# jedward225/MARL-HideAndSeek

Measured on AMD Instinct MI355X. Metric: world-steps/sec (agent-steps/sec derived) at 16K worlds, 1/2/4/8 GPU, higher is better.
Workload: dtype f32; 1 GPU; 16000 worlds/GPU x 2646 steps, 2 hiders + 2 seekers, sim_flags=0, rand_seed=0, random move actions in [-5,4] each step (scripts/benchmark.py args); worlds_per_gpu=16000, total_worlds=16000, agents_per_world=4

## Files before the change

### marl-hideandseek_amd/csrc/hs_k_physics.h

```cpp
#pragma once
#include "hs_state.h"
#include "hs_rays.h"
#include "hs_collide.h"
#include "hs_solver.h"
#include "hs_k_reset.h"

namespace hs {

constexpr int kPhysThreads = 64;
constexpr int kWorldLanes = kPhysThreads / kTile;
constexpr int kLdsWalls = 32;
static_assert(kMaxSCand <= 32 && kMaxDDCand <= 16, "accepted-manifold masks are one word per world");
constexpr int kAllDD = kNumDSlots * (kNumDSlots - 1) / 2;
constexpr int kAllSC = kNumDSlots * (kMaxWalls + kMaxPlanes - 1);
constexpr int kSpInfoWords = kNumDSlots + 1;

struct alignas(16) OctRes {
    static constexpr int kClip = kClipLanes;
    static constexpr int kClipWords = clip_words(kClip);
    static constexpr int kSatPairs = kClip < hs::kSatPairs ? kClip : hs::kSatPairs;
    static constexpr int kMaxItems = kTile * (kMaxDDCand + kMaxSCand);
    static constexpr int kSlots = kClip < 31 ? kClip : 31;
    static constexpr int kVelOffsetWords = 2 * 8 * 3 * 32;
    float pos[3][kNumDSlots][kTile];
    float rot[4][kNumDSlots][kTile];
    float ppos[3][kNumDSlots][kTile];
    float prot[4][kNumDSlots][kTile];
    int meta[kNumDSlots][kTile];
    union {
        struct {
            float lo[3][kNumDSlots][kTile], hi[3][kNumDSlots][kTile];
            float wall[4][kLdsWalls][kTile];
        } det;
        struct {
            float clip[kClipWords];
            unsigned short items[kMaxItems + 32];
            int pend[4][kClip];
        } sat;
        struct {
            float pad[kVelOffsetWords];
            float lin[3][kNumDSlots][kTile];
            float ang[3][kNumDSlots][kTile];
        } vel;
    } u;
    unsigned short ddPair[kMaxDDCand][kTile];
    unsigned short scPair[kMaxSCand][kTile];
    unsigned short scInfo[kNumDSlots][kTile];
    unsigned int scAcc[kTile];
    unsigned int ddAcc[kTile];
    unsigned int ddOrd[2][kTile];
    float plane0[4][kTile];
    unsigned char bodies[kNumDSlots * kTile];
    union {
        unsigned char wallBodies[kNumDSlots * kTile];
        unsigned char actGL[kMaxAgents][kTile];
    };
    unsigned int wallSeen[kTile];
    unsigned char numWalls[kTile], numPlanes[kTile], ndd[kTile], nsc[kTile], seen[kTile], hasGrab[kTile];
    unsigned char spill[kTile];
    int wid[kTile];
};
constexpr int kSeenDeferred = 2;
static_assert(sizeof(OctRes) <= 20 * 1024, "8 waves of 8 worlds share the CU's 160 KiB of LDS");
static_assert(offsetof(OctRes, u.sat.items) >= offsetof(OctRes, u.det.wall), "items must not overlap the AABBs");
static_assert(sizeof(ManDD) / 4 * OctRes::kSlots <= OctRes::kVelOffsetWords, "manifold slots lie below the velocities");
static_assert(2 * 3 * kNumDSlots * 8 <= OctRes::kVelOffsetWords, "the hull AABBs lie below the velocities");

constexpr int kLocGlobal = 31;
HSD int pair_a(int p) { return p & 31; }
HSD int pair_b(int p) { return (p >> 5) & 63; }
HSD int pair_loc(int p) { return (p >> 11) & 31; }
HSD int pair_pack(int a, int b) { return a | (b << 5) | (kLocGlobal << 11); }
static_assert(kNumDSlots <= 32 && kMaxWalls + kMaxPlanes <= 64, "pair encoding");
static_assert(sizeof(ManDD) % 16 == 0 && sizeof(ManS) % 16 == 0, "manifold records move 16 bytes at a time");
constexpr int kManWords = sizeof(ManDD) / 4;
template <typename M> HSD void man_lds_load(const float *clip, int slot, M &m) {
    m = *reinterpret_cast<const M *>(clip + slot * kManWords);
}
template <typename M> HSD void man_lds_set_lam(float *clip, int slot, int j, float v) {
    static_assert(offsetof(M, lam) == sizeof(M) - 16, "lam is the record's tail");
    clip[slot * kManWords + (sizeof(M) / 4 - 4 + j)] = v;
}

template <int C> HSD V3 rld3(const float (&a)[C][kNumDSlots][kTile], int slot, int g) { return {a[0][slot][g], a[1][slot][g], a[2][slot][g]}; }
HSD Q rld4(const float (&a)[4][kNumDSlots][kTile], int slot, int g) { return {a[0][slot][g], a[1][slot][g], a[2][slot][g], a[3][slot][g]}; }
HSD void rst3(float (&a)[3][kNumDSlots][kTile], int slot, int g, V3 v) { a[0][slot][g] = v.x; a[1][slot][g] = v.y; a[2][slot][g] = v.z; }
HSD void rst4(float (&a)[4][kNumDSlots][kTile], int slot, int g, Q q) { a[0][slot][g] = q.w; a[1][slot][g] = q.x; a[2][slot][g] = q.y; a[3][slot][g] = q.z; }

HSD void rbody_load(const OctRes &R, int g, int slot, BodyS &b) {
    b.pos = rld3(R.pos, slot, g); b.rot = rld4(R.rot, slot, g);
    b.ppos = rld3(R.ppos, slot, g); b.prot = rld4(R.prot, slot, g);
    b.lin = rld3(R.u.vel.lin, slot, g); b.ang = rld3(R.u.vel.ang, slot, g);
    const int m = R.meta[slot][g];
    const bool dyn = m != 0 && meta_resp(m) == RESP_DYNAMIC;
    b.invM = dyn ? obj_inv_mass(meta_obj(m)) : 0.f;
    b.invI = dyn ? obj_inv_inertia(meta_obj(m)) : V3{0.f, 0.f, 0.f};
    body_refresh_inertia(b);
}
HSD void rbody_store_pose(OctRes &R, int g, int slot, const BodyS &b) { rst3(R.pos, slot, g, b.pos); rst4(R.rot, slot, g, b.rot); }
HSD void rbody_store_vel(OctRes &R, int g, int slot, const BodyS &b) { rst3(R.u.vel.lin, slot, g, b.lin); rst3(R.u.vel.ang, slot, g, b.ang); }
HSD void derive_velocity(BodyS &b) {
    const float h = kSubstepH;
    b.lin = (b.pos - b.ppos) * (1.f / h);
    Q dq = qmul(b.rot, qinv(b.prot));
    V3 wv = V3{dq.x, dq.y, dq.z} * (2.f / h);
    b.ang = dq.w >= 0.f ? wv : -wv;
}

HSD void wave_sync() { asm volatile("s_waitcnt lgkmcnt(0)" ::: "memory"); }
HSD void mem_sync() { asm volatile("s_waitcnt vmcnt(0) lgkmcnt(0)" ::: "memory"); }

template <int D> HSD int dpp_row_shr(int x) { return __builtin_amdgcn_update_dpp(0, x, 0x110 + D, 0xF, 0xF, true); }
HSD int scan8_incl(int x, int l) {
    int y;
    y = dpp_row_shr<1>(x); if (l >= 1) x += y;
    y = dpp_row_shr<2>(x); if (l >= 2) x += y;
    y = dpp_row_shr<4>(x); if (l >= 4) x += y;
    return x;
}
HSD int sum8_all(int x) {
    x += __builtin_amdgcn_update_dpp(0, x, 0xB1, 0xF, 0xF, false);
    x += __builtin_amdgcn_update_dpp(0, x, 0x4E, 0xF, 0xF, false);
    x += __builtin_amdgcn_update_dpp(0, x, 0x141, 0xF, 0xF, false);
    return x;
}
HSD int scan64_incl(int x) {
    x += dpp_row_shr<1>(x); x += dpp_row_shr<2>(x); x += dpp_row_shr<4>(x); x += dpp_row_shr<8>(x);
    x += __builtin_amdgcn_update_dpp(0, x, 0x142, 0xA, 0xF, false);
    x += __builtin_amdgcn_update_dpp(0, x, 0x143, 0xC, 0xF, false);
    return x;
}

struct ResGeom {
    const OctRes &R; const SimState &S; int g; int w;
    HSD int g_meta(int i) const { return R.meta[i][g]; }
    HSD V3 g_pos(int i) const { return rld3(R.pos, i, g); }
    HSD Q g_rot(int i) const { return rld4(R.rot, i, g); }
    HSD int g_num_walls() const { return R.numWalls[g]; }
    HSD float g_wall(int k, int c) const { return S.walls(c * kMaxWalls + k, w); }
    HSD int g_num_planes() const { return R.numPlanes[g]; }
    HSD float g_plane(int p, int c) const { return S.planes(c * kMaxPlanes + p, w); }
};

constexpr float kGroundOff = 0.f;
struct BodyReg {
    int np, vidx;
    float lam[4];
};

template <typename E, int ROWS>
HSD void copy_in(E *dst, const Col<E, ROWS> &col, int p0) {
    static_assert(sizeof(E) == 4, "16-byte pieces");
    const float4 *src = reinterpret_cast<const float4 *>(col.octet(p0 >> 3));
    float4 *d = reinterpret_cast<float4 *>(dst);
    for (int i = hs_lane(); i < ROWS * 2; i += 64) d[i] = src[(i / 2) * 2 + i % 2];
}
template <typename E, int ROWS>
HSD void copy_out(const Col<E, ROWS> &col, int p0, const E *src) {
    static_assert(sizeof(E) == 4, "16-byte pieces");
    float4 *dst = reinterpret_cast<float4 *>(col.octet(p0 >> 3));
    const float4 *s = reinterpret_cast<const float4 *>(src);
    for (int i = hs_lane(); i < ROWS * 2; i += 64) dst[(i / 2) * 2 + i % 2] = s[i];
}
HSD void copy_out_vel(const Col<float, 3 * kNumDSlots> &col, int p0, const float *src, const OctRes &R) {
    float *dst = col.octet(p0 >> 3);
    for (int i = hs_lane(); i < 3 * kNumDSlots * kTile; i += 64) {
        const int row = i / kTile, g = i % kTile, slot = row % kNumDSlots;
        const int m = R.meta[slot][g];
        if (m != 0 && meta_resp(m) == RESP_DYNAMIC) dst[row * kTile + g] = src[i];
    }
}

HSD void integrate_body(OctRes &R, BodyReg &b, int slot, int g, int meta, const float *aforce) {
    const int obj = meta_obj(meta);
    const bool dyn = meta_resp(meta) == RESP_DYNAMIC;
    V3 force = {0.f, 0.f, 0.f}; float torque = 0.f;
    if (dyn && slot >= kAgentSlot0) {
        const float *f = aforce + (slot - kAgentSlot0) * kTile + g;
        force = {f[0 * kMaxAgents * kTile], f[1 * kMaxAgents * kTile], f[2 * kMaxAgents * kTile]};
        torque = f[3 * kMaxAgents * kTile];
    }
    V3 pos = rld3(R.pos, slot, g); Q rot = rld4(R.rot, slot, g);
    rst3(R.ppos, slot, g, pos); rst4(R.prot, slot, g, rot);
    if (dyn) {
        V3 lin = rld3(R.u.vel.lin, slot, g), ang = rld3(R.u.vel.ang, slot, g);
        const float h = kSubstepH;
        const float invM = obj_inv_mass(obj);
        const V3 invI = obj_inv_inertia(obj);
        lin = madd(lin, madd(V3{0.f, 0.f, kGravityZ}, force, invM), h);
        pos = madd(pos, lin, h);
        Q qi = qinv(rot);
        V3 wloc = qrot(qi, ang), tl = qrot(qi, V3{0.f, 0.f, torque});
        const V3 I = obj_inertia(obj);
        V3 Iw = mulc(I, wloc);
        wloc = madd(wloc, mulc(invI, tl - cross(wloc, Iw)), h);
        ang = qrot(rot, wloc);
        rot = quat_add_rotation(rot, ang * h);
        rst3(R.pos, slot, g, pos); rst4(R.rot, slot, g, rot);
        rst3(R.u.vel.lin, slot, g, lin); rst3(R.u.vel.ang, slot, g, ang);
    }
    V3 lo, hi;
    const HullRef hb = hull_ref_body(obj, pos, rot);
    hull_aabb(hb, &lo, &hi);
    rst3(R.u.det.lo, slot, g, lo); rst3(R.u.det.hi, slot, g, hi);
    b.np = 0; b.vidx = 0;
#pragma unroll
    for (int j = 0; j < 4; ++j) b.lam[j] = 0.f;
    if (dyn && R.numPlanes[g] >= 1) {
        const V3 pn = {R.plane0[0][g], R.plane0[1][g], R.plane0[2][g]};
        b.np = ground_manifold(hb, pn, R.plane0[3][g], &b.vidx);
    }
}

struct ItemCounts { int nbox, nwedge; bool anySpill; };
template <int JB>
HSD ItemCounts phase_detect(const SimState &S, OctRes &R, int NS) {
    constexpr int G = kWorldLanes;
    const int L = hs_lane(), g = L / G, l = L % G;
    {
        constexpr int PR = kTile / 4;
        static_assert(kLdsWalls * PR <= 64, "one piece per lane per component");
        const float *src = S.walls.octet(S.wbeg >> 3);
        float4 v[4];
        const bool on = L < kLdsWalls * PR;
        const int row = L / PR, part = L % PR;
#pragma unroll
        for (int c = 0; c < 4; ++c) if (on) v[c] = *(const float4 *)(src + (c * kMaxWalls + row) * kTile + 4 * part);
#pragma unroll
        for (int c = 0; c < 4; ++c) if (on) *(float4 *)(&R.u.det.wall[c][row][4 * part]) = v[c];
    }
    if (l == 0) { R.scAcc[g] = 0u; R.ddAcc[g] = 0u; }
    wave_sync();
    const int nwl = R.numWalls[g], npl = R.numPlanes[g];
    int tot_items = 0;
    unsigned dd_mask[JB] = {}; unsigned long long s_mask[JB] = {};
    int bdd[JB] = {}, bsc[JB] = {}, add[JB] = {}, asc[JB] = {};
    bool have[JB], dynamic[JB]; V3 lo[JB], hi[JB];
#pragma unroll
    for (int jb = 0; jb < JB; ++jb) {
        const int slot = l + jb * G;
        const int meta = slot < NS ? R.meta[slot][g] : 0;
        have[jb] = meta != 0;
        dynamic[jb] = have[jb] && meta_resp(meta) == RESP_DYNAMIC;
        lo[jb] = {0.f, 0.f, 0.f}; hi[jb] = {0.f, 0.f, 0.f};
        if (have[jb]) { lo[jb] = rld3(R.u.det.lo, slot, g); hi[jb] = rld3(R.u.det.hi, slot, g); }
    }
#pragma unroll 4
    for (int j = 1; j < NS; ++j) {
        const int mj = R.meta[j][g];
        const bool dynj = meta_resp(mj) == RESP_DYNAMIC;
        const V3 loj = rld3(R.u.det.lo, j, g), hij = rld3(R.u.det.hi, j, g);
#pragma unroll
        for (int jb = 0; jb < JB; ++jb) {
            const bool hit = (mj != 0) & have[jb] & (l + jb * G < j) & (dynamic[jb] | dynj) &
                (lo[jb].x <= hij.x) & (loj.x <= hi[jb].x) & (lo[jb].y <= hij.y) & (loj.y <= hi[jb].y) &
                (lo[jb].z <= hij.z) & (loj.z <= hi[jb].z);
            dd_mask[jb] |= hit ? 1u << j : 0u;
        }
    }
    bool zin[JB];
#pragma unroll
    for (int jb = 0; jb < JB; ++jb) zin[jb] = dynamic[jb] & (lo[jb].z <= 2.5f) & (0.f <= hi[jb].z);
    auto wall_test = [&](int k, float cx, float cy, float hx, float hy) {
        const float wx0 = cx - hx, wx1 = cx + hx, wy0 = cy - hy, wy1 = cy + hy;
#pragma unroll
        for (int jb = 0; jb < JB; ++jb) {
            const bool hit = zin[jb] & (lo[jb].x <= wx1) & (wx0 <= hi[jb].x) & (lo[jb].y <= wy1) & (wy0 <= hi[jb].y);
            s_mask[jb] |= hit ? 1ull << k : 0ull;
        }
    };
    const int nwLds = nwl < kLdsWalls ? nwl : kLdsWalls;
#pragma unroll 4
    for (int k = 0; k < nwLds; ++k) wall_test(k, R.u.det.wall[0][k][g], R.u.det.wall[1][k][g], R.u.det.wall[2][k][g], R.u.det.wall[3][k][g]);
    for (int k = kLdsWalls; k < nwl; ++k) {
        const int w = S.wbeg + g;
        wall_test(k, S.walls(0 * kMaxWalls + k, w), S.walls(1 * kMaxWalls + k, w), S.walls(2 * kMaxWalls + k, w), S.walls(3 * kMaxWalls + k, w));
    }
    int tot_dd = 0, tot_sc = 0;
#pragma unroll
    for (int jb = 0; jb < JB; ++jb) {
        if (dynamic[jb]) for (int p = 1; p < npl; ++p) s_mask[jb] |= 1ull << (kMaxWalls + p);
        const int cdd = __popc(dd_mask[jb]), csc = __popcll(s_mask[jb]);
        const int in_dd = scan8_incl(cdd, l), in_sc = scan8_incl(csc, l);
        bdd[jb] = tot_dd + in_dd - cdd; bsc[jb] = tot_sc + in_sc - csc;
        tot_dd += sum8_all(cdd); tot_sc += sum8_all(csc);
        add[jb] = cdd ? max(0, min(cdd, kMaxDDCand - bdd[jb])) : 0;
        asc[jb] = csc ? max(0, min(csc, kMaxSCand - bsc[jb])) : 0;
        tot_items += add[jb] + asc[jb];
        if (add[jb] != cdd) atomicAdd(&S.status[0], cdd - add[jb]);
        if (asc[jb] != csc) atomicAdd(&S.status[1], csc - asc[jb]);
    }
    const bool spillDD = tot_dd > kMaxDDCand, spillSC = tot_sc > kMaxSCand;
    const bool anySpill = __ballot(spillDD || spillSC) != 0ull;
    unsigned short *const spPair = S.spPair + (size_t)(S.wbeg + g) * (kAllDD + kAllSC);
    int *const spInfo = S.spInfo + (size_t)(S.wbeg + g) * kSpInfoWords;
    int n_wedge = 0;
#pragma unroll
    for (int jb = 0; jb < JB; ++jb) {
        const int slot = l + jb * G;
        const bool ramp = slot >= kRampSlot0 && slot < kRampSlot0 + kMaxRamps;
        if (ramp) n_wedge += add[jb] + asc[jb];
        else { unsigned mm = dd_mask[jb]; for (int i = 0; mm && i < add[jb]; ++i) { const int j = __ffs(mm) - 1; mm &= mm - 1; n_wedge += (j >= kRampSlot0 && j < kRampSlot0 + kMaxRamps) ? 1 : 0; } }
    }
    const int n_box = tot_items - n_wedge;
    const int inc_box = scan64_incl(n_box), inc_wedge = scan64_incl(n_wedge);
    ItemCounts ic;
    ic.anySpill = anySpill;
    ic.nbox = __builtin_amdgcn_readlane(inc_box, 63); ic.nwedge = __builtin_amdgcn_readlane(inc_wedge, 63);
    const int wedge0 = (ic.nbox + 31) / 32 * 32;
    int ibox = inc_box - n_box, iwedge = wedge0 + inc_wedge - n_wedge;
    wave_sync();
#pragma unroll
    for (int jb = 0; jb < JB; ++jb) {
        const int slot = l + jb * G;
        const bool ramp = slot >= kRampSlot0 && slot < kRampSlot0 + kMaxRamps;
        unsigned mm = dd_mask[jb]; int i = 0;
        while (mm && i < add[jb]) {
            const int j = __ffs(mm) - 1; mm &= mm - 1;
            R.ddPair[bdd[jb] + i][g] = (unsigned short)pair_pack(slot, j);
            const unsigned short item = (unsigned short)((g << 6) | (bdd[jb] + i));
            if (ramp || (j >= kRampSlot0 && j < kRampSlot0 + kMaxRamps)) R.u.sat.items[iwedge++] = item; else R.u.sat.items[ibox++] = item;
            ++i;
        }
        while (mm) {
            const int j = __ffs(mm) - 1; mm &= mm - 1;
            spPair[bdd[jb] + i] = (unsigned short)pair_pack(slot, j);
            ++i;
        }
        unsigned long long sm = (s_mask[jb] >> kMaxWalls) | (s_mask[jb] << (64 - kMaxWalls) >> (64 - kMaxWalls) << kMaxPlanes); i = 0;
        while (sm && i < asc[jb]) {
            const int bit = __ffsll((long long)sm) - 1; sm &= sm - 1;
            const int k = bit < kMaxPlanes ? kMaxWalls + bit : bit - kMaxPlanes;
            R.scPair[bsc[jb] + i][g] = (unsigned short)pair_pack(slot, k);
            const unsigned short item = (unsigned short)((g << 6) | 32 | (bsc[jb] + i));
            if (ramp) R.u.sat.items[iwedge++] = item; else R.u.sat.items[ibox++] = item;
            ++i;
        }
        const int nspill = sm ? __popcll(sm) : 0;
        while (sm) {
            const int bit = __ffsll((long long)sm) - 1; sm &= sm - 1;
            const int k = bit < kMaxPlanes ? kMaxWalls + bit : bit - kMaxPlanes;
            spPair[kAllDD + bsc[jb] + i] = (unsigned short)pair_pack(slot, k);
            ++i;
        }
        if (spillSC && slot < kNumDSlots) spInfo[1 + slot] = nspill ? ((bsc[jb] + asc[jb]) | (nspill << 16)) : 0;
        if (slot < NS) R.scInfo[slot][g] = (unsigned short)(asc[jb] > 0 ? (bsc[jb] | (asc[jb] << 8)) : 0);
    }
    if (l == 0) {
        R.spill[g] = (unsigned char)((spillDD ? 1 : 0) | (spillSC ? 2 : 0));
        if (spillDD || spillSC) spInfo[0] = tot_dd | (tot_sc << 16);
        R.ndd[g] = (unsigned char)min(tot_dd, kMaxDDCand); R.nsc[g] = (unsigned char)min(tot_sc, kMaxSCand);
        if (R.wid[g] >= 0 && tot_dd + tot_sc > 0) S.loadAcc[R.wid[g]] += tot_dd + tot_sc;
    }
    wave_sync();
    return ic;
}

template <bool POS, int UNROLL, typename SetLam>
HSD void static_manifold(BodyS &me, const ManS &m, SetLam set_lam) {
    BodyS none;
    body_refresh_inertia(me);
    const V3 n = ld3(m.n);
    const int np = m.np;
    const float mu = POS ? m.muS : m.muD;
#pragma unroll UNROLL
    for (int j = 0; j < 4; ++j)
        if (j < np) {
            const float lamj = m.lam[j];
            if (POS) set_lam(j, lamj + solve_point_position<false>(me, none, n, ld3(m.rA[j]), V3{0.f, 0.f, 0.f}, m.offB[j], mu));
            else solve_point_velocity<false>(me, none, n, ld3(m.rA[j]), V3{0.f, 0.f, 0.f}, lamj, mu);
        }
}

#define HS_COLD __device__ __forceinline__
struct SpillCtx {
    const float *walls, *planes;
    ManDD *wsDD; ManS *wsSC; unsigned short *spPair; int *spInfo;
    int wbeg;
};
HSD SpillCtx spill_ctx(const SimState &S) { return {S.walls.p, S.planes.p, (ManDD *)S.wsDD, (ManS *)S.wsSC, S.spPair, S.spInfo, S.wbeg}; }

HS_COLD void spill_sat(SpillCtx c, OctRes *Rp) {
    OctRes &R = *Rp;
    const int lane = hs_lane() & 63;
    const bool hi = (lane & 1) != 0;
    const Col<float, 4 * kMaxWalls> walls = {const_cast<float *>(c.walls)};
    const Col<float, 4 * kMaxPlanes> planes = {const_cast<float *>(c.planes)};
#pragma unroll 1
    for (int g = 0; g < kTile; ++g) {
        const int fl = __builtin_amdgcn_readfirstlane((int)R.spill[g]);
        if (fl == 0) continue;
        const int w = c.wbeg + g;
        const int tot = __builtin_amdgcn_readfirstlane(c.spInfo[(size_t)w * kSpInfoWords]);
#pragma unroll 1
        for (int kind = 0; kind < 2; ++kind) {
            if ((fl & (1 << kind)) == 0) continue;
            const bool isdd = kind == 0;
            const int n = isdd ? tot & 0xffff : tot >> 16;
#pragma unroll 1
            for (int base = isdd ? kMaxDDCand : kMaxSCand; base < n; base += OctRes::kSatPairs) {
                const int kk = base + (lane >> 1);
                if (kk < n && (lane >> 1) < OctRes::kSatPairs) {
                    const int pair = c.spPair[(size_t)w * (kAllDD + kAllSC) + (isdd ? 0 : kAllDD) + kk];
                    const int a = pair_a(pair), bsel = pair_b(pair);
                    const int oa = meta_obj(R.meta[a][g]);
                    const V3 pa = rld3(R.pos, a, g);
                    const Q qa = rld4(R.rot, a, g);
                    ManDD *const md = c.wsDD + (size_t)w * kAllDD + kk;
                    ManS *const ms = c.wsSC + (size_t)w * kAllSC + kk;
                    RawManifold raw;
                    raw.np = 0;
                    bool plane = false;
                    if (!isdd && bsel >= kMaxWalls) {
                        const int p = bsel - kMaxWalls;
                        const V3 pn = {planes(0 * kMaxPlanes + p, w), planes(1 * kMaxPlanes + p, w), planes(2 * kMaxPlanes + p, w)};
                        plane = true;
                        if (!hi && !collide_hull_plane(hull_ref_body(oa, pa, qa), pn, planes(3 * kMaxPlanes + p, w), raw)) raw.np = 0;
                    } else {
                        const HullSrc ha = hull_src_body(oa, pa, qa);
                        const HullSrc hb = isdd ? hull_src_body(meta_obj(R.meta[bsel][g]), rld3(R.pos, bsel, g), rld4(R.rot, bsel, g))
                                                : hull_src_wall(walls(0 * kMaxWalls + bsel, w), walls(1 * kMaxWalls + bsel, w),
                                                                walls(2 * kMaxWalls + bsel, w), walls(3 * kMaxWalls + bsel, w));
                        const AxisResult res = sat_axes(ha, hb, hi);
                        const ClipBuf cb = {R.u.sat.clip, lane >> 1, OctRes::kClip};
                        if (!hi && res.code != 0 && !sat_contact(ha, hb, res, cb, raw)) raw.np = 0;
                    }
                    if (!hi) {
                        const int ob = isdd ? meta_obj(R.meta[bsel][g]) : plane ? OBJ_PLANE : OBJ_WALL;
                        const float muS = 0.5f * (obj_mu_s(oa) + obj_mu_s(ob)), muD = 0.5f * (obj_mu_d(oa) + obj_mu_d(ob));
                        const Q qai = qinv(qa);
                        if (isdd) {
                            md->a = a; md->b = bsel; md->np = raw.np; md->muS = muS; md->muD = muD;
                            st3(md->n, raw.n);
                            const V3 pb = rld3(R.pos, bsel, g);
                            const Q qbi = qinv(rld4(R.rot, bsel, g));
#pragma unroll
                            for (int j = 0; j < 4; ++j)
                                if (j < raw.np) {
                                    st3(md->rA[j], qrot(qai, raw.pA[j] - pa)); st3(md->rB[j], qrot(qbi, raw.pB[j] - pb));
                                    md->lam[j] = 0.f;
                                }
                        } else {
                            ms->np = raw.np; ms->muS = muS; ms->muD = muD;
                            st3(ms->n, raw.n);
#pragma unroll
                            for (int j = 0; j < 4; ++j)
                                if (j < raw.np) {
                                    st3(ms->rA[j], plane ? hull_local_vertex(oa, raw.vidx[j]) : qrot(qai, raw.pA[j] - pa));
                                    ms->offB[j] = dot(raw.pB[j], raw.n); ms->lam[j] = 0.f;
                                }
                        }
                    }
                }
                wave_sync();
            }
        }
    }
    mem_sync();
}

template <bool POS>
HS_COLD void spill_dd(SpillCtx c, OctRes *Rp) {
    OctRes &R = *Rp;
#pragma unroll 1
    for (int g = 0; g < kTile; ++g) {
        if ((__builtin_amdgcn_readfirstlane((int)R.spill[g]) & 1) == 0) continue;
        const int w = c.wbeg + g;
        const int nall = __builtin_amdgcn_readfirstlane(c.spInfo[(size_t)w * kSpInfoWords]) & 0xffff;
        if (hs_lane() == 0) {
#pragma unroll 1
            for (int k = kMaxDDCand; k < nall; ++k) {
                ManDD *const m = c.wsDD + (size_t)w * kAllDD + k;
                const int np = m->np;
                if (np <= 0) continue;
                const int ba = m->a, bb = m->b;
                BodyS Ab, Bb;
                rbody_load(R, g, ba, Ab); rbody_load(R, g, bb, Bb);
                const V3 n = ld3(m->n);
                const float mu = POS ? m->muS : m->muD;
#pragma unroll 1
                for (int j = 0; j < np; ++j) {
                    const float lamj = m->lam[j];
                    if (POS) m->lam[j] = lamj + solve_point_position<true>(Ab, Bb, n, ld3(m->rA[j]), ld3(m->rB[j]), 0.f, mu);
                    else solve_point_velocity<true>(Ab, Bb, n, ld3(m->rA[j]), ld3(m->rB[j]), lamj, mu);
                }
                if (POS) { rbody_store_pose(R, g, ba, Ab); rbody_store_pose(R, g, bb, Bb); }
                else { rbody_store_vel(R, g, ba, Ab); rbody_store_vel(R, g, bb, Bb); }
                wave_sync();
            }
        }
    }
}

template <bool POS>
HS_COLD void spill_static(SpillCtx c, OctRes *Rp, int NS) {
    OctRes &R = *Rp;
#pragma unroll 1
    for (int g = 0; g < kTile; ++g) {
        if ((__builtin_amdgcn_readfirstlane((int)R.spill[g]) & 2) == 0) continue;
        const int w = c.wbeg + g;
        const int slot = hs_lane();
        if (slot >= NS) continue;
        const int info = c.spInfo[(size_t)w * kSpInfoWords + 1 + slot];
        const int first = info & 0xffff, cnt = info >> 16;
        if (cnt == 0) continue;
        BodyS me;
        rbody_load(R, g, slot, me);
#pragma unroll 1
        for (int k = first; k < first + cnt; ++k) {
            ManS &m = c.wsSC[(size_t)w * kAllSC + k];
            if (m.np <= 0) continue;
            static_manifold<POS, 1>(me, m, [&](int j, float v) { m.lam[j] = v; });
        }
        if (POS) rbody_store_pose(R, g, slot, me); else rbody_store_vel(R, g, slot, me);
    }
}

HSD HullSrc sat_hull_a(const OctRes &R, int g, int a) { return hull_src_body(meta_obj(R.meta[a][g]), rld3(R.pos, a, g), rld4(R.rot, a, g)); }
HSD HullSrc sat_hull_b(const SimState &S, const OctRes &R, int g, int w, bool isdd, int bsel) {
    if (isdd) return hull_src_body(meta_obj(R.meta[bsel][g]), rld3(R.pos, bsel, g), rld4(R.rot, bsel, g));
    return hull_src_wall(S.walls(0 * kMaxWalls + bsel, w), S.walls(1 * kMaxWalls + bsel, w),
                         S.walls(2 * kMaxWalls + bsel, w), S.walls(3 * kMaxWalls + bsel, w));
}
HSD bool sat_flush(const SimState &S, OctRes &R, int npend, bool last) {
    const int lane = hs_lane() & 63;
    const bool toLds = last && lane < OctRes::kSlots;
    bool wroteGlobal = false;
    int mw[kManWords]; int mkind = 0, mkk = 0, mg = 0, mpair = 0;
    if (lane < npend) {
        const int item = R.u.sat.pend[0][lane] & 0xffff;
        AxisResult res;
        res.code = R.u.sat.pend[0][lane] >> 16;
        res.ax = {__int_as_float(R.u.sat.pend[1][lane]), __int_as_float(R.u.sat.pend[2][lane]), __int_as_float(R.u.sat.pend[3][lane])};
        const int g = item >> 6, idx = item & 63;
        const int w = S.wbeg + g;
        const bool isdd = idx < 32;
        const int kk = idx & 31;
        const int pair = isdd ? R.ddPair[kk][g] : R.scPair[kk][g];
        const int a = pair_a(pair), bsel = pair_b(pair);
        const ClipBuf cb = {R.u.sat.clip, lane, OctRes::kClip};
        RawManifold raw;
        const bool plane = res.code == 3;
        bool have;
        if (plane) {
            const int p = bsel - kMaxWalls;
            const V3 pn = {S.planes(0 * kMaxPlanes + p, w), S.planes(1 * kMaxPlanes + p, w), S.planes(2 * kMaxPlanes + p, w)};
            have = collide_hull_plane(hull_ref_body(meta_obj(R.meta[a][g]), rld3(R.pos, a, g), rld4(R.rot, a, g)), pn, S.planes(3 * kMaxPlanes + p, w), raw);
        } else {
            have = sat_contact(sat_hull_a(R, g, a), sat_hull_b(S, R, g, w, isdd, bsel), res, cb, raw);
        }
        if (have) {
            const int oa = meta_obj(R.meta[a][g]);
            const int ob = isdd ? meta_obj(R.meta[bsel][g]) : plane ? OBJ_PLANE : OBJ_WALL;
            const V3 pa = rld3(R.pos, a, g);
            const Q qai = qinv(rld4(R.rot, a, g));
            const float muS = 0.5f * (obj_mu_s(oa) + obj_mu_s(ob)), muD = 0.5f * (obj_mu_d(oa) + obj_mu_d(ob));
            if (isdd) {
                ManDD m;
                m.a = a; m.b = bsel; m.np = raw.np; m.muS = muS; m.muD = muD;
                st3(m.n, raw.n);
                const V3 pb = rld3(R.pos, bsel, g);
                const Q qbi = qinv(rld4(R.rot, bsel, g));
#pragma unroll
                for (int j = 0; j < 4; ++j) {
                    const bool on = j < raw.np;
                    st3(m.rA[j], on ? qrot(qai, raw.pA[j] - pa) : V3{0.f, 0.f, 0.f});
                    st3(m.rB[j], on ? qrot(qbi, raw.pB[j] - pb) : V3{0.f, 0.f, 0.f});
                    m.lam[j] = 0.f;
                }
                if (toLds) { __builtin_memcpy(mw, &m, sizeof(m)); mkind = 1; mkk = kk; mg = g; mpair = pair; }
                else { ((ManDD *)S.wsDD + (size_t)w * kAllDD)[kk] = m; wroteGlobal = true; }
                atomicOr(&R.ddAcc[g], 1u << kk);
            } else {
                ManS m;
                m.np = raw.np; m.muS = muS; m.muD = muD; m.pad[0] = 0.f; m.pad[1] = 0.f;
                st3(m.n, raw.n);
#pragma unroll
                for (int j = 0; j < 4; ++j) {
                    const bool on = j < raw.np;
// ... 452 lines not shown
                } else if (owner == OWNER_NONE) {
                    R.meta[hit][g] = meta_pack(obj, RESP_STATIC, type == AGENT_HIDER ? OWNER_HIDER : OWNER_SEEKER);
                }
            }
        }
        if (fl & 1) {
            if (S.grabOther(i, w) >= 0) {
                S.grabOther(i, w) = -1;
            } else {
                float t; V3 o = mpos + V3{0.f, 0.f, 0.5f};
                V3 dir = qrot(mrot, {0.f, 1.f, 0.f});
                int hit = trace_ray(geom, o, dir, 2.5f, &t);
                if (hit >= 0 && hit < kNumDSlots) {
                    const int m = R.meta[hit][g];
                    if (meta_owner(m) == OWNER_NONE && meta_resp(m) == RESP_DYNAMIC) {
                        V3 hit_pos = o + dir * t;
                        Q erot = geom.g_rot(hit);
                        V3 r2 = qrot(qinv(erot), hit_pos - geom.g_pos(hit));
                        Q at2 = qnormalize(qmul(qinv(erot), mrot));
                        S.grabOther(i, w) = hit;
                        const float gd[kGrabWords] = {r2.x, r2.y, r2.z, at2.w, at2.x, at2.y, at2.z, t - 1.25f,
                                                      0.f, 1.25f, 0.5f,
                                                      1.f, 0.f, 0.f, 0.f};
#pragma unroll
                        for (int c = 0; c < kGrabWords; ++c) S.grabData(c * kMaxAgents + i, w) = gd[c];
                    }
                }
            }
        }
    }
}

HSD void phase_pre(const SimState &S, OctRes &R) {
    const int A_ = S.A, L = hs_lane();
    const bool instant = (S.flags & FLAG_ZERO_AGENT_VELOCITY) == FLAG_ZERO_AGENT_VELOCITY;
    bool need_action = false;
    if (L < kMaxAgents * kTile) {
        const int agent = L / kTile, g = L % kTile;
        const int w = R.wid[g], p = S.wbeg + g;
        int fl = 0;
        if (agent < A_ && w >= 0) {
            const int teams = S.teams[w], step = S.curEpisodeStep[w];
            const bool active = team_agent_active(teams, agent) != 0;
            const int type = team_agent_type(teams, agent);
            if (active && !(type == AGENT_SEEKER && step < kNumPrepSteps - 1)) {
                int32_t *act_row = S.xAction + (w * A_ + agent) * 5;
                const int ax = act_row[0], ay = act_row[1], ar = act_row[2], ag = act_row[3], al = act_row[4];
                float fx, fy, tz;
                if (instant) { fx = 400.f * (float)(ax - 2); fy = 400.f * (float)(ay - 2); tz = 120.f * (float)(ar - 2); }
                else { fx = 12.f * (float)(ax - 5); fy = 12.f * (float)(ay - 5); tz = 3.f * (float)(ar - 5); }
                V3 f = qrot(rld4(R.rot, kAgentSlot0 + agent, g), {fx, fy, 0.f});
                S.aforce(0 * kMaxAgents + agent, p) = f.x; S.aforce(1 * kMaxAgents + agent, p) = f.y;
                S.aforce(2 * kMaxAgents + agent, p) = f.z; S.aforce(3 * kMaxAgents + agent, p) = tz;
                fl = (ag == 1 ? 1 : 0) | (al == 1 ? 2 : 0);
                act_row[0] = 2; act_row[1] = 2; act_row[2] = 2; act_row[3] = 0; act_row[4] = 0;
            }
        }
        R.actGL[agent][g] = (unsigned char)fl;
        need_action = fl != 0;
    }
    const bool any = __ballot(need_action) != 0ull;
    wave_sync();
    if (any && L < kTile && R.wid[L] >= 0) {
        bool want = false;
        for (int a = 0; a < A_; ++a) want |= R.actGL[a][L] != 0;
        if (want) action_system(S, R, L, A_, S.teams[R.wid[L]]);
    }
    if (L < kTile) {
        bool grab = false;
        if (R.wid[L] >= 0) for (int a = 0; a < kMaxAgents; ++a) grab |= S.grabOther(a, S.wbeg + L) >= 0;
        R.hasGrab[L] = grab ? 1 : 0;
    }
    wave_sync();
}

HSD void phase_post(const SimState &S, OctRes &R) {
    constexpr int G = kWorldLanes;
    const int L = hs_lane(), g = L / G, l = L % G;
    const int w = R.wid[g], p = S.wbeg + g;
    const int A_ = S.A;
    const bool wok = w >= 0;
    const bool instant = (S.flags & FLAG_ZERO_AGENT_VELOCITY) == FLAG_ZERO_AGENT_VELOCITY;
    int teams = 0, step = 0, counts = 0, resetReq = 0;
    float hider_reward = 0.f;
    if (wok) {
        teams = S.teams[w]; step = S.curEpisodeStep[w]; counts = S.counts[w];
        hider_reward = S.hiderTeamReward[w]; resetReq = S.xReset[w];
        if (l == 0) R.seen[g] = 0;
        if (instant && l < kMaxAgents && R.meta[kAgentSlot0 + l][g] != 0) {
            const int slot = kAgentSlot0 + l;
            R.u.vel.lin[0][slot][g] = 0.f; R.u.vel.lin[1][slot][g] = 0.f;
            R.u.vel.lin[2][slot][g] = fminf(R.u.vel.lin[2][slot][g], 0.f);
            rst3(R.u.vel.ang, slot, g, V3{0.f, 0.f, 0.f});
        }
    }
    const bool undecided = wok && step >= kNumPrepSteps - 1 && hider_reward != -1.f;
    const bool defer = undecided && (S.flags & FLAG_EXT_SKIP_OBSERVATIONS) != FLAG_EXT_SKIP_OBSERVATIONS && resetReq == 0 &&
                       !((S.flags & FLAG_IGNORE_EPISODE_LENGTH) != FLAG_IGNORE_EPISODE_LENGTH && step == kEpisodeLen - 1);
    if (defer && l == 0) R.seen[g] = kSeenDeferred;
    wave_sync();
    for (int pr = l; undecided && !defer && pr < 9; pr += G) {
        const int si = pr / 3, hi_ = pr % 3;
        if (si < cnt_seekers(counts) && hi_ < cnt_hiders(counts)) {
            const ResGeom geom = {R, S, g, p};
            const int ss = kAgentSlot0 + team_seeker(teams, si), hs_ = kAgentSlot0 + team_hider(teams, hi_);
            const V3 spos = geom.g_pos(ss);
            const V3 fwd = qrot(geom.g_rot(ss), {0.f, 1.f, 0.f});
            V3 to = geom.g_pos(hs_) - spos;
            float c = dot(normalize(to), fwd);
            if (!(c < kCosFovHalf)) {
                float t;
                if (trace_ray(geom, spos, to, 1.f, &t) == hs_) R.seen[g] = 1;
            }
        }
    }
    wave_sync();
    if (!wok) return;
    if (R.seen[g] == 1) hider_reward = -1.f;
    if (l < A_ && team_agent_active(teams, l)) {
        const int agent = l, slot = kAgentSlot0 + agent, row = w * A_ + agent;
        if (step == 0) S.xDone[row] = 0;
        if (step < kNumPrepSteps - 1) {
            S.xReward[row] = 0.f;
        } else {
            if (step == kEpisodeLen - 1) S.xDone[row] = 1;
            float r = hider_reward;
            if (team_agent_type(teams, agent) == AGENT_SEEKER) r *= -1.f;
            if (fabsf(R.pos[0][slot][g]) >= 18.f || fabsf(R.pos[1][slot][g]) >= 18.f) r -= 10.f;
            S.xReward[row] = r;
        }
    }
    if (l == 0) {
        float *res = S.xEpisodeResult + w * 2;
        int s0 = S.runningScores(0, p), s1 = S.runningScores(1, p);
        if (step == 0) { res[0] = 0.f; res[1] = 0.f; s0 = 0; s1 = 0; }
        if (step >= kNumPrepSteps) {
            const bool hidden = hider_reward == 1.f;
            const bool sf = cnt_seekers_first(counts) != 0;
            const int win = hidden ? (sf ? 1 : 0) : (sf ? 0 : 1);
            if (win == 0) s0 += 1; else s1 += 1;
        }
        if (step == kEpisodeLen - 1) {
            if (s0 > s1) { res[0] = 1.f; res[1] = 0.f; }
            else if (s0 < s1) { res[0] = 0.f; res[1] = 1.f; }
            else { res[0] = 0.5f; res[1] = 0.5f; }
        }
        S.runningScores(0, p) = s0; S.runningScores(1, p) = s1;
        S.hiderTeamReward[w] = hider_reward;
    }
}

template <int ROUNDS, int LASTR, bool POS>
HSD void static_passes(const SimState &S, OctRes &R, BodyReg (&br)[ROUNDS], int nbodies, int nLast, int nMerged) {
    const int L = hs_lane();
#pragma unroll
    for (int r = 0; r < LASTR; ++r) {
        const bool valid = r * 64 + L < nbodies; const int t_ = valid ? R.bodies[r * 64 + L] : 0;
        const int slot = t_ >> 3, g = t_ & 7; const int meta = valid ? R.meta[slot][g] : 0;
        if (valid) { if (POS) ground_pos(R, br[r], slot, g, meta); else ground_vel(R, br[r], slot, g, meta); }
    }
    wave_sync();
    {
        const bool valid = LASTR * 64 + L < nbodies; const int t_ = valid ? R.bodies[LASTR * 64 + L] : 0;
        const int slot = t_ >> 3, g = t_ & 7; const int meta = valid ? R.meta[slot][g] : 0;
        last_round<POS>(S, R, br[LASTR], valid, slot, g, meta, nLast, nMerged);
    }
    wave_sync();
}

#ifdef HS_PHASE_TIMING
#define HS_TICK_PARAMS , long long &tk, long long (&acc)[10]
#define HS_TICK_ARGS , tk, acc
#define HS_TICK(i) { const long long now_ = wall_clock64(); acc[i] += now_ - tk; tk = now_; }
#else
#define HS_TICK_PARAMS
#define HS_TICK_ARGS
#define HS_TICK(i)
#endif
#define HS_BODY(r) const bool valid = (r) * 64 + L < nbodies; const int t_ = valid ? R.bodies[(r) * 64 + L] : 0; \
                   const int slot = t_ >> 3, g = t_ & 7; const int meta = valid ? R.meta[slot][g] : 0;
template <int ROUNDS>
HSD void substep_rest(const SimState &S, OctRes &R, BodyReg (&br)[ROUNDS], int nbodies, int NS, ItemCounts ic, bool integrateNext,
                      const float *aforce HS_TICK_PARAMS) {
    const int L = hs_lane();
    const bool manGlobal = phase_sat(S, R, ic);
    HS_TICK(3)
    phase_dd<true>(S, R, ic.anySpill);
    HS_TICK(4)
    constexpr int kShortLastR = ROUNDS - 2;
    const bool shortLast = ROUNDS == 3 && nbodies <= 64 * (ROUNDS - 1);
    const int lastRound = shortLast ? kShortLastR : ROUNDS - 1;
    const WallLists wl = list_wall_bodies<ROUNDS>(R, nbodies, lastRound);
    const int nLast = max(nbodies - 64 * lastRound, 0);
    const int nMerged = min(wl.nEarly, 64 - nLast);
    if (shortLast) static_passes<ROUNDS, kShortLastR, true>(S, R, br, nbodies, nLast, nMerged);
    else static_passes<ROUNDS, ROUNDS - 1, true>(S, R, br, nbodies, nLast, nMerged);
    if (wl.nwb > nMerged) { wall_round<true>(S, R, nMerged, wl.nwb); wave_sync(); }
    if (__builtin_expect(ic.anySpill, 0)) { spill_static<true>(spill_ctx(S), &R, NS); wave_sync(); }
#pragma unroll
    for (int r = 0; r < ROUNDS; ++r) { HS_BODY(r) if (valid) derive_body_velocity(R, slot, g, meta); }
    if (manGlobal) mem_sync(); else wave_sync();
    HS_TICK(5)
    phase_dd<false>(S, R, ic.anySpill);
    HS_TICK(6)
    if (shortLast) static_passes<ROUNDS, kShortLastR, false>(S, R, br, nbodies, nLast, nMerged);
    else static_passes<ROUNDS, ROUNDS - 1, false>(S, R, br, nbodies, nLast, nMerged);
    if (wl.nwb > nMerged) { wall_round<false>(S, R, nMerged, wl.nwb); wave_sync(); }
    if (__builtin_expect(ic.anySpill, 0)) { spill_static<false>(spill_ctx(S), &R, NS); wave_sync(); }
    if (integrateNext) {
#pragma unroll
        for (int r = 0; r < ROUNDS; ++r) { HS_BODY(r) if (valid) integrate_body(R, br[r], slot, g, meta, aforce); }
        wave_sync();
    }
    HS_TICK(7)
}

template <int ROUNDS>
HSD void physics_step(SimState &S, OctRes &R, GenScratch *gen) {
    const int L = hs_lane();
    const int noct = gridDim.x;
    const int sidx = step_ring(S), prevIdx = sidx == 0 ? 2 : sidx - 1, nextIdx = sidx == 2 ? 0 : sidx + 1;
    const int serve = step_serve(S);
    if (serve != kGroupEarly && blockIdx.x == 0 && L == 0) {
        S.tickSum[nextIdx] = 0ull;
        atomicExch(group_count(S, prevIdx, kGroupEarly), 0); atomicExch(group_count(S, prevIdx, kGroupLate), 0);
    }
    int o = blockIdx.x;
    if (serve != kGroupAll) {
        if (o >= *group_count(S, sidx, serve)) return;
        o = oct_list(S, sidx, serve, noct)[o];
    }
    S.wbeg = o * kTile;
    const int p0 = S.wbeg;
    const int NS = kAgentSlot0 + S.A;
    const long long tStart = wall_clock64();
    int prevTicks, lateAbove;
    {
        prevTicks = S.octTicks[o];
        const float mean = (float)S.tickSum[prevIdx] / (float)noct, mine = (float)prevTicks;
        const bool known = mean > 0.f;
        lateAbove = __builtin_amdgcn_readfirstlane(known ? (int)fminf(2.f * __int_as_float(sched_words(S)[kSchedFactor]) * mean, 2.0e9f) : 0x7fffffff);
        const bool late = serve == kGroupLate;
        if (late && L == 0) atomicAdd(&S.status[2], 1);
        if (known && mine > 1.10f * mean) __builtin_amdgcn_s_setprio(3);
        else if (known && mine > 0.98f * mean) __builtin_amdgcn_s_setprio(2);
        else if ((known && mine > 0.88f * mean) || (known && late)) __builtin_amdgcn_s_setprio(1);
        else if (known) __builtin_amdgcn_s_setprio(0);
        else __builtin_amdgcn_s_setprio(2);
    }
#ifdef HS_PHASE_TIMING
    long long tk = wall_clock64(); long long acc[10] = {0, 0, 0, 0, 0, 0, 0, 0, 0, 0};
#endif
    copy_in(&R.pos[0][0][0], S.bpos, p0); copy_in(&R.rot[0][0][0], S.brot, p0);
    copy_in(&R.u.vel.lin[0][0][0], S.blin, p0); copy_in(&R.u.vel.ang[0][0][0], S.bang, p0);
    copy_in(&R.meta[0][0], S.bmeta, p0);
    if (L < kTile) {
        const int w = S.worldOfSlot[S.wbeg + L];
        R.wid[L] = w;
        R.numWalls[L] = w >= 0 ? (unsigned char)S.numWalls[w] : 0;
        R.numPlanes[L] = w >= 0 ? (unsigned char)S.numPlanes[w] : 0;
        R.seen[L] = 0; R.ndd[L] = 0; R.nsc[L] = 0;
        R.wallSeen[L] = w >= 0 ? (unsigned)S.wallHist[w] : 0u;
    }
    if (L < 4 * kTile) (&R.plane0[0][0])[L] = S.planes((L / kTile) * kMaxPlanes, S.wbeg + (L % kTile));
    wave_sync();
    HS_TICK(9)
    phase_pre(S, R);
    HS_TICK(0)
    int nbodies;
    {
        int base = 0;
#pragma unroll
        for (int pass = 0; pass < 2; ++pass) {
#pragma unroll
            for (int c = 0; c < ROUNDS; ++c) {
                const int t = c * 64 + L;
                const int ord = t / kTile, g = t % kTile;
                const int slot = ord < S.A ? kAgentSlot0 + ord : ord - S.A;
                const bool hist = ord < NS && ((R.wallSeen[g] >> slot) & 1u) != 0u;
                const bool on = ord < NS && R.meta[slot][g] != 0 && hist == (pass == 0);
                const unsigned long long m = __ballot(on);
                if (on) R.bodies[base + __popcll(m & ((1ull << L) - 1ull))] = (unsigned char)(slot << 3 | g);
                base += __popcll(m);
            }
        }
        nbodies = base;
    }
    wave_sync();
    if (L < kTile) R.wallSeen[L] = 0u;
    wave_sync();
    BodyReg br[ROUNDS];
    const float *const aforce = S.aforce.octet(p0 >> 3);
#pragma unroll
    for (int r = 0; r < ROUNDS; ++r) {
        BodyReg &b = br[r];
        b.np = 0; b.vidx = 0;
#pragma unroll
        for (int j = 0; j < 4; ++j) b.lam[j] = 0.f;
        HS_BODY(r)
        if (valid) integrate_body(R, b, slot, g, meta, aforce);
    }
    wave_sync();
    HS_TICK(1)
#pragma unroll 1
    for (int sub = 0; sub < kNumSubsteps; ++sub) {
        const ItemCounts ic = phase_detect<ROUNDS>(S, R, NS);
        HS_TICK(2)
        substep_rest<ROUNDS>(S, R, br, nbodies, NS, ic, sub + 1 < kNumSubsteps, aforce HS_TICK_ARGS);
    }
#undef HS_BODY
    phase_post(S, R);
    wave_sync();
    copy_out(S.bpos, p0, &R.pos[0][0][0]); copy_out(S.brot, p0, &R.rot[0][0][0]);
    copy_out_vel(S.blin, p0, &R.u.vel.lin[0][0][0], R); copy_out_vel(S.bang, p0, &R.u.vel.ang[0][0][0], R);
    copy_out(S.bmeta, p0, &R.meta[0][0]);
    mem_sync();
    HS_TICK(8)
    {
        const int myWorld = L < kTile ? R.wid[L] : -1;
        const int mySeen = L < kTile ? (int)R.wallSeen[L] : 0;
        const bool myDeferred = L < kTile && R.seen[L] == kSeenDeferred;
        wave_sync();
        if (myWorld >= 0) {
            S.wallHist[myWorld] = mySeen;
            reset_world(S, myWorld, gen[L], myDeferred);
        }
    }
    if (L == 0) {
        const int dt = (int)(wall_clock64() - tStart);
        S.octTicks[o] = dt;
        atomicAdd(&S.tickSum[sidx], (unsigned long long)dt);
        const int group = dt + prevTicks > lateAbove ? kGroupLate : kGroupEarly;
        oct_list(S, nextIdx, group, noct)[atomicAdd(group_count(S, nextIdx, group), 1)] = o;
    }
#ifdef HS_PHASE_TIMING
    if (L == 0) for (int i = 0; i < 10; ++i) S.phaseTicks[(size_t)o * 10 + i] += acc[i];
#endif
#undef HS_TICK
}

template <int ROUNDS>
__global__ void __launch_bounds__(kPhysThreads, 2) k_physics(SimState S) {
    __shared__ union PhysLds { OctRes R; GenScratch gen[kTile]; } lds;
    static_assert(sizeof(PhysLds) <= 20 * 1024, "8 waves of 8 worlds share the CU's 160 KiB of LDS");
    physics_step<ROUNDS>(S, lds.R, lds.gen);
}

}
```

Measured before the change: 34.61 million world-steps/s.

## Use strip-binned wall culling and half-sweep pair tests in broadphase

Replaces the full O(N^2) body-pair AABB sweep with a cyclic half-distance sweep: each lane tests only about half the offsets and shares hits through LDS atomicOr exchange masks. Wall tests are culled with per-world 8-strip x/y bitmasks, precomputed once per step and broadcast via ds_bpermute, so only candidate walls get an exact box test. Wall staging is split into an early global load and a deferred LDS store to overlap latency. The risks are added atomics, extra permutes and data-dependent loops, and strip culling gives no saving when walls span many strips.

```diff
diff --git a/marl-hideandseek_amd/csrc/hs_broadphase.h b/marl-hideandseek_amd/csrc/hs_broadphase.h
--- /dev/null
+++ b/marl-hideandseek_amd/csrc/hs_broadphase.h
@@ -0,0 +1,36 @@
+#pragma once
+#include "hs_core.h"
+
+namespace hs {
+
+constexpr int kStrips = 8;
+
+HSD int strip_of(float v) {
+    const float t = v * 0.2f + 4.f;
+    return (int)__builtin_fminf(__builtin_fmaxf(t, 0.f), (float)(kStrips - 1));
+}
+HSD unsigned strip_range(int a, int b) {
+    const int lo = a < b ? a : b, hi = a < b ? b : a;
+    return (2u << hi) - (1u << lo);
+}
+HSD unsigned extent_strips(float v0, float v1) { return strip_range(strip_of(v0), strip_of(v1)); }
+
+struct WallBox { float x0, x1, y0, y1; };
+HSD WallBox wall_box(float cx, float cy, float hx, float hy) { return {cx - hx, cx + hx, cy - hy, cy + hy}; }
+HSD bool wall_hit(bool zin, float lox, float hix, float loy, float hiy, WallBox w) {
+    return zin & (lox <= w.x1) & (w.x0 <= hix) & (loy <= w.y1) & (w.y0 <= hiy);
+}
+HSD unsigned wall_strips(float cx, float cy, float hx, float hy) {
+    const WallBox w = wall_box(cx, cy, hx, hy);
+    return extent_strips(w.x0, w.x1) | (extent_strips(w.y0, w.y1) << 8);
+}
+HSD unsigned strip_mask_part(unsigned w, int s, int j) { return ((w >> s) & 0x01010101u) << j; }
+
+HSD bool aabb_hit(V3 loa, V3 hia, V3 lob, V3 hib) {
+    return (loa.x <= hib.x) & (lob.x <= hia.x) & (loa.y <= hib.y) & (lob.y <= hia.y) & (loa.z <= hib.z) & (lob.z <= hia.z);
+}
+HSD int pair_steps(int ns) { return ns >> 1; }
+HSD bool pair_mine(int s, int d, int ns) { return 2 * d != ns || s < d; }
+HSD int pair_next(int j, int ns) { return j + 1 == ns ? 0 : j + 1; }
+
+}
diff --git a/marl-hideandseek_amd/csrc/hs_k_physics.h b/marl-hideandseek_amd/csrc/hs_k_physics.h
--- a/marl-hideandseek_amd/csrc/hs_k_physics.h
+++ b/marl-hideandseek_amd/csrc/hs_k_physics.h
@@ -3,6 +3,7 @@
 #include "hs_rays.h"
 #include "hs_collide.h"
 #include "hs_solver.h"
+#include "hs_broadphase.h"
 #include "hs_k_reset.h"
 
 namespace hs {
@@ -31,6 +32,7 @@
         struct {
             float lo[3][kNumDSlots][kTile], hi[3][kNumDSlots][kTile];
             float wall[4][kLdsWalls][kTile];
+            unsigned xch[kNumDSlots][kTile];
         } det;
         struct {
             float clip[kClipWords];
@@ -63,6 +65,7 @@
 constexpr int kSeenDeferred = 2;
 static_assert(sizeof(OctRes) <= 20 * 1024, "8 waves of 8 worlds share the CU's 160 KiB of LDS");
 static_assert(offsetof(OctRes, u.sat.items) >= offsetof(OctRes, u.det.wall), "items must not overlap the AABBs");
+static_assert(sizeof(decltype(OctRes::u.det)) <= sizeof(decltype(OctRes::u.sat)), "the broadphase scratch adds nothing to the octet's LDS");
 static_assert(sizeof(ManDD) / 4 * OctRes::kSlots <= OctRes::kVelOffsetWords, "manifold slots lie below the velocities");
 static_assert(2 * 3 * kNumDSlots * 8 <= OctRes::kVelOffsetWords, "the hull AABBs lie below the velocities");
 
@@ -212,24 +215,53 @@
     }
 }
 
+typedef float WallPiece __attribute__((ext_vector_type(4)));
+struct WallPieces { WallPiece cx, cy, hx, hy; };
+static_assert(kLdsWalls * (kTile / 4) == kPhysThreads, "one 16-byte piece per lane and component");
+HSD WallPieces stage_walls_load(const SimState &S) {
+    const int L = hs_lane();
+    const float *src = S.walls.octet(S.wbeg >> 3) + 4 * L;
+    return {*(const WallPiece *)(src + 0 * kMaxWalls * kTile), *(const WallPiece *)(src + 1 * kMaxWalls * kTile),
+            *(const WallPiece *)(src + 2 * kMaxWalls * kTile), *(const WallPiece *)(src + 3 * kMaxWalls * kTile)};
+}
+HSD void stage_walls_store(OctRes &R, const WallPieces &p) {
+    const int L = hs_lane();
+    *(WallPiece *)(&R.u.det.wall[0][0][0] + 4 * L) = p.cx; *(WallPiece *)(&R.u.det.wall[1][0][0] + 4 * L) = p.cy;
+    *(WallPiece *)(&R.u.det.wall[2][0][0] + 4 * L) = p.hx; *(WallPiece *)(&R.u.det.wall[3][0][0] + 4 * L) = p.hy;
+}
+HSD void issue_fence() { __builtin_amdgcn_sched_barrier(0); }
+HSD int world_lane0() { return (hs_lane() & ~(kWorldLanes - 1)) * 4; }
+HSD unsigned world_lane(unsigned x, int lane0, int s) { return (unsigned)__builtin_amdgcn_ds_bpermute(lane0 + s * 4, (int)x); }
+HSD void wall_strip_masks(const OctRes &R, unsigned &xm, unsigned &ym) {
+    static_assert(kLdsWalls == 4 * kWorldLanes && kStrips == kWorldLanes, "a byte of strips per wall, four walls per lane");
+    const int L = hs_lane(), g = L / kWorldLanes, l = L % kWorldLanes;
+    const int nw = R.numWalls[g];
+    unsigned wx = 0u, wy = 0u;
+#pragma unroll
+    for (int r = 0; r < 4; ++r) {
+        const int k = l + r * kWorldLanes;
+        const unsigned b = wall_strips(R.u.det.wall[0][k][g], R.u.det.wall[1][k][g], R.u.det.wall[2][k][g], R.u.det.wall[3][k][g]);
+        wx |= k < nw ? (b & 0xffu) << (8 * r) : 0u;
+        wy |= k < nw ? (b >> 8) << (8 * r) : 0u;
+    }
+    xm = 0u; ym = 0u;
+    const int lane0 = world_lane0();
+    unsigned fx[kWorldLanes], fy[kWorldLanes];
+#pragma unroll
+    for (int j = 0; j < kWorldLanes; ++j) { fx[j] = world_lane(wx, lane0, j); fy[j] = world_lane(wy, lane0, j); }
+    issue_fence();
+#pragma unroll
+    for (int j = 0; j < kWorldLanes; ++j) { xm |= strip_mask_part(fx[j], l, j); ym |= strip_mask_part(fy[j], l, j); }
+}
 struct ItemCounts { int nbox, nwedge; bool anySpill; };
 template <int JB>
-HSD ItemCounts phase_detect(const SimState &S, OctRes &R, int NS) {
+HSD ItemCounts phase_detect(const SimState &S, OctRes &R, int NS, unsigned xm, unsigned ym) {
     constexpr int G = kWorldLanes;
     const int L = hs_lane(), g = L / G, l = L % G;
-    {
-        constexpr int PR = kTile / 4;
-        static_assert(kLdsWalls * PR <= 64, "one piece per lane per component");
-        const float *src = S.walls.octet(S.wbeg >> 3);
-        float4 v[4];
-        const bool on = L < kLdsWalls * PR;
-        const int row = L / PR, part = L % PR;
-#pragma unroll
-        for (int c = 0; c < 4; ++c) if (on) v[c] = *(const float4 *)(src + (c * kMaxWalls + row) * kTile + 4 * part);
-#pragma unroll
-        for (int c = 0; c < 4; ++c) if (on) *(float4 *)(&R.u.det.wall[c][row][4 * part]) = v[c];
-    }
+    const WallPieces wp = stage_walls_load(S);
     if (l == 0) { R.scAcc[g] = 0u; R.ddAcc[g] = 0u; }
+#pragma unroll
+    for (int jb = 0; jb < JB; ++jb) if (l + jb * G < kNumDSlots) R.u.det.xch[l + jb * G][g] = 0u;
     wave_sync();
     const int nwl = R.numWalls[g], npl = R.numPlanes[g];
     int tot_items = 0;
@@ -245,36 +277,108 @@
         lo[jb] = {0.f, 0.f, 0.f}; hi[jb] = {0.f, 0.f, 0.f};
         if (have[jb]) { lo[jb] = rld3(R.u.det.lo, slot, g); hi[jb] = rld3(R.u.det.hi, slot, g); }
     }
-#pragma unroll 4
-    for (int j = 1; j < NS; ++j) {
-        const int mj = R.meta[j][g];
-        const bool dynj = meta_resp(mj) == RESP_DYNAMIC;
-        const V3 loj = rld3(R.u.det.lo, j, g), hij = rld3(R.u.det.hi, j, g);
+    {
+        int pj[JB]; unsigned hm[JB];
+#pragma unroll
+        for (int jb = 0; jb < JB; ++jb) { pj[jb] = have[jb] ? l + jb * G : 0; hm[jb] = 0u; }
+        const int nd = pair_steps(NS);
+        for (int d = 1; d <= nd; d += 2) {
+            int pjs[2][JB], mj[2][JB]; V3 loj[2][JB], hij[2][JB];
+#pragma unroll
+            for (int u = 0; u < 2; ++u)
+#pragma unroll
+                for (int jb = 0; jb < JB; ++jb) {
+                    const int j = pair_next(pj[jb], NS);
+                    pj[jb] = j; pjs[u][jb] = j;
+                    mj[u][jb] = R.meta[j][g];
+                    loj[u][jb] = rld3(R.u.det.lo, j, g); hij[u][jb] = rld3(R.u.det.hi, j, g);
+                }
+            issue_fence();
+#pragma unroll
+            for (int u = 0; u < 2; ++u)
+#pragma unroll
+                for (int jb = 0; jb < JB; ++jb) {
+                    const bool dynj = meta_resp(mj[u][jb]) == RESP_DYNAMIC;
+                    const bool hit = (d + u <= nd) & (mj[u][jb] != 0) & have[jb] & pair_mine(l + jb * G, d + u, NS) & (dynamic[jb] | dynj) &
+                        aabb_hit(lo[jb], hi[jb], loj[u][jb], hij[u][jb]);
+                    hm[jb] |= hit ? 1u << pjs[u][jb] : 0u;
+                }
+        }
 #pragma unroll
         for (int jb = 0; jb < JB; ++jb) {
-            const bool hit = (mj != 0) & have[jb] & (l + jb * G < j) & (dynamic[jb] | dynj) &
-                (lo[jb].x <= hij.x) & (loj.x <= hi[jb].x) & (lo[jb].y <= hij.y) & (loj.y <= hi[jb].y) &
-                (lo[jb].z <= hij.z) & (loj.z <= hi[jb].z);
-            dd_mask[jb] |= hit ? 1u << j : 0u;
+            const int slot = l + jb * G;
+            unsigned below = hm[jb] & ((1u << slot) - 1u);
+            while (below) {
+                const int j = __ffs(below) - 1; below &= below - 1;
+                atomicOr(&R.u.det.xch[j][g], 1u << slot);
+            }
+        }
+        stage_walls_store(R, wp);
+        wave_sync();
+#pragma unroll
+        for (int jb = 0; jb < JB; ++jb) {
+            const int slot = l + jb * G;
+            dd_mask[jb] = (hm[jb] & ~((2u << slot) - 1u)) | (slot < kNumDSlots ? R.u.det.xch[slot][g] : 0u);
         }
     }
     bool zin[JB];
+    unsigned wcand[JB], whit[JB];
 #pragma unroll
     for (int jb = 0; jb < JB; ++jb) zin[jb] = dynamic[jb] & (lo[jb].z <= 2.5f) & (0.f <= hi[jb].z);
-    auto wall_test = [&](int k, float cx, float cy, float hx, float hy) {
-        const float wx0 = cx - hx, wx1 = cx + hx, wy0 = cy - hy, wy1 = cy + hy;
+    {
+        unsigned sx[JB], sy[JB], ax[JB], ay[JB];
 #pragma unroll
         for (int jb = 0; jb < JB; ++jb) {
-            const bool hit = zin[jb] & (lo[jb].x <= wx1) & (wx0 <= hi[jb].x) & (lo[jb].y <= wy1) & (wy0 <= hi[jb].y);
-            s_mask[jb] |= hit ? 1ull << k : 0ull;
-        }
-    };
-    const int nwLds = nwl < kLdsWalls ? nwl : kLdsWalls;
-#pragma unroll 4
-    for (int k = 0; k < nwLds; ++k) wall_test(k, R.u.det.wall[0][k][g], R.u.det.wall[1][k][g], R.u.det.wall[2][k][g], R.u.det.wall[3][k][g]);
+            sx[jb] = extent_strips(lo[jb].x, hi[jb].x); sy[jb] = extent_strips(lo[jb].y, hi[jb].y);
+            ax[jb] = 0u; ay[jb] = 0u;
+        }
+        const int lane0 = world_lane0();
+        unsigned mx[kStrips], my[kStrips];
+#pragma unroll
+        for (int s = 0; s < kStrips; ++s) { mx[s] = world_lane(xm, lane0, s); my[s] = world_lane(ym, lane0, s); }
+        issue_fence();
+#pragma unroll
+        for (int s = 0; s < kStrips; ++s)
+#pragma unroll
+            for (int jb = 0; jb < JB; ++jb) { ax[jb] |= (sx[jb] >> s & 1u) ? mx[s] : 0u; ay[jb] |= (sy[jb] >> s & 1u) ? my[s] : 0u; }
+#pragma unroll
+        for (int jb = 0; jb < JB; ++jb) { wcand[jb] = zin[jb] ? ax[jb] & ay[jb] : 0u; whit[jb] = 0u; }
+    }
+    for (;;) {
+        unsigned left = 0u;
+#pragma unroll
+        for (int jb = 0; jb < JB; ++jb) left |= wcand[jb];
+        if (left == 0u) break;
+        int wk[2][JB]; bool won[2][JB]; float wv[2][JB][4];
+#pragma unroll
+        for (int u = 0; u < 2; ++u)
+#pragma unroll
+            for (int jb = 0; jb < JB; ++jb) {
+                const unsigned m = wcand[jb];
+                const int k = (__ffs(m) - 1) & (kLdsWalls - 1);
+                wcand[jb] = m & (m - 1u);
+                wk[u][jb] = k; won[u][jb] = m != 0u;
+#pragma unroll
+                for (int c = 0; c < 4; ++c) wv[u][jb][c] = R.u.det.wall[c][k][g];
+            }
+        issue_fence();
+#pragma unroll
+        for (int u = 0; u < 2; ++u)
+#pragma unroll
+            for (int jb = 0; jb < JB; ++jb) {
+                const WallBox wb = wall_box(wv[u][jb][0], wv[u][jb][1], wv[u][jb][2], wv[u][jb][3]);
+                const bool hit = won[u][jb] & wall_hit(zin[jb], lo[jb].x, hi[jb].x, lo[jb].y, hi[jb].y, wb);
+                whit[jb] |= hit ? 1u << wk[u][jb] : 0u;
+            }
+    }
+#pragma unroll
+    for (int jb = 0; jb < JB; ++jb) s_mask[jb] = whit[jb];
     for (int k = kLdsWalls; k < nwl; ++k) {
         const int w = S.wbeg + g;
-        wall_test(k, S.walls(0 * kMaxWalls + k, w), S.walls(1 * kMaxWalls + k, w), S.walls(2 * kMaxWalls + k, w), S.walls(3 * kMaxWalls + k, w));
+        const WallBox wb = wall_box(S.walls(0 * kMaxWalls + k, w), S.walls(1 * kMaxWalls + k, w), S.walls(2 * kMaxWalls + k, w), S.walls(3 * kMaxWalls + k, w));
+#pragma unroll
+        for (int jb = 0; jb < JB; ++jb)
+            s_mask[jb] |= wall_hit(zin[jb], lo[jb].x, hi[jb].x, lo[jb].y, hi[jb].y, wb) ? 1ull << k : 0ull;
     }
     int tot_dd = 0, tot_sc = 0;
 #pragma unroll
@@ -1333,9 +1437,13 @@
     }
     wave_sync();
     HS_TICK(1)
+    unsigned wallsX, wallsY;
+    stage_walls_store(R, stage_walls_load(S));
+    wave_sync();
+    wall_strip_masks(R, wallsX, wallsY);
 #pragma unroll 1
     for (int sub = 0; sub < kNumSubsteps; ++sub) {
-        const ItemCounts ic = phase_detect<ROUNDS>(S, R, NS);
+        const ItemCounts ic = phase_detect<ROUNDS>(S, R, NS, wallsX, wallsY);
         HS_TICK(2)
         substep_rest<ROUNDS>(S, R, br, nbodies, NS, ic, sub + 1 < kNumSubsteps, aforce HS_TICK_ARGS);
     }
```

Result: faster. 35.23 million world-steps/s (median of 6 runs) (+1.8%).
